# zypher-game/uzkge

Hardware: AMD Instinct MI355X
Metric: bn254_g1_msm_points_per_sec (higher is better)
Workload: dtype u256 (254-bit modular integers: 8 x u32 Montgomery limbs in HBM, 9 x 29-bit limbs in the two hot loops); 1 GPU; BN254 G1 MSM, 2^24 random points + uniform scalars per GPU, bases resident in HBM; points_per_gpu=16777216, total_points=16777216

## Files before the change

### uzkge_amd/csrc/api.cpp

```cpp
#include <algorithm>
#include <atomic>
#include <cstdarg>
#include <cstdlib>
#include <cstring>
#include <exception>
#include <new>
#include <vector>

#include "anemoi29.hpp"
#include "ctx.hpp"
#include "lane_tools.hpp"
#include "fq12_29.hpp"
#include "g16_pk_layout.hpp"
#include "g2_29.hpp"
#include "host_ec64.hpp"
#include "host_math.hpp"
#include "shufflecs_dev.hpp"
#include "matchcs_dev.hpp"

namespace uzk {

static thread_local char g_err[512] = "";

void set_error(const char* fmt, ...) {
// ... 281 lines not shown
    prover_release_all();
    vf_release_all();
    g2_release_all();
    rcs_release_all();
    g16_release_all();
    g16v_release_all();
    remark_release_all();
    std::lock_guard<std::mutex> lk(s.mu);
    if (!s.bound) return UZK_OK;
    ctx_release(default_ctx());
    for (auto& kv : s.contexts) { ctx_release(*kv.second); delete kv.second; }
    s.contexts.clear();
    s.epoch.fetch_add(1, std::memory_order_acq_rel);
    t_handle = 0;
    t_cached = nullptr;
    for (auto& kv : s.srs) {
        (void)hipSetDevice(kv.second.device);
        if (kv.second.owned && kv.second.d_points) (void)hipFree(kv.second.d_points);
        if (kv.second.d_table) (void)hipFree(kv.second.d_table);
    }
    s.srs.clear();
    s.num_cus.clear();
    s.bound = false;
    s.device = -1;
    return UZK_OK;
} catch (...) { return uzk::on_exception("uzk_shutdown"); }

namespace uzk {
static void copy_tuning(const Ctx& from, Ctx& to) {
    to.msm_window_bits = from.msm_window_bits;
    to.tune_no_precompute = from.tune_no_precompute; to.tune_ntt_tile = from.tune_ntt_tile; to.tune_ntt_two_pass = from.tune_ntt_two_pass; to.tune_small = from.tune_small;
    to.tune_chunk_log = from.tune_chunk_log; to.tune_verify_transcript = from.tune_verify_transcript; to.tune_stream_log = from.tune_stream_log; to.tune_stream_min_log = from.tune_stream_min_log;
    to.tune_seg_sort = from.tune_seg_sort; to.tune_arith29 = from.tune_arith29;
    to.tune_msm_taper = from.tune_msm_taper;
}
}
int uzk_ctx_create(uint64_t* ctx_out) try {
    if (!ctx_out) { set_error("uzk_ctx_create: null pointer"); return UZK_ERR_PARAMETER; }
    Ctx* c = new Ctx();
    {
        API_LOCK;
        int rc = require_ready();
        if (rc != UZK_OK) { delete c; return rc; }
        copy_tuning(ctx(), *c);
    }
    Shared& s = shared();
    std::lock_guard<std::mutex> lk(s.mu);
    const uint64_t h = s.next_ctx++;
    s.contexts[h] = c;
    *ctx_out = h;
    return UZK_OK;
} catch (...) { return uzk::on_exception("uzk_ctx_create"); }
int uzk_ctx_create_on(int device, uint64_t* ctx_out) try {
    if (!ctx_out) { set_error("uzk_ctx_create_on: null pointer"); return UZK_ERR_PARAMETER; }
    int n = 0;
    if (hipGetDeviceCount(&n) != hipSuccess || n <= 0) { set_error("no HIP device visible: the MI355X backend has no CPU fallback"); return UZK_ERR_DEVICE; }
    if (device < 0 || device >= n) { set_error("uzk_ctx_create_on(%d): %d device(s) visible", device, n); return UZK_ERR_PARAMETER; }
    Ctx* c = new Ctx();
    {
        API_LOCK;
        copy_tuning(ctx(), *c);
    }
    c->want_device = device;
    Shared& s = shared();
    std::lock_guard<std::mutex> lk(s.mu);
    const uint64_t h = s.next_ctx++;
    s.contexts[h] = c;
// ... 1874 lines not shown
    UZK_HIP(hipStreamSynchronize(ctx().stream));
    return UZK_OK;
} catch (...) { return uzk::on_exception("uzk_sync"); }
void* uzk_stream(void) {
    API_LOCK;
    if (require_ready() != UZK_OK) return nullptr;
    return ctx().stream;
}
int uzk_msm_set_window_bits(int c) try {
    API_LOCK;
    if (c != 0 && (c < 4 || c > 22)) { set_error("window bits must be 0 (auto) or 4..22"); return UZK_ERR_PARAMETER; }
    ctx().msm_window_bits = c;
    return UZK_OK;
} catch (...) { return uzk::on_exception("uzk_msm_set_window_bits"); }

int uzk_msm_plan_info(size_t n, int* window_bits, int* windows) try {
    API_LOCK;
    if (!window_bits || !windows || n == 0) { set_error("uzk_msm_plan_info: bad arguments"); return UZK_ERR_PARAMETER; }
    msm_plan_info(ctx(), n, window_bits, windows);
    return UZK_OK;
} catch (...) { return uzk::on_exception("uzk_msm_plan_info"); }

int uzk_tune(const char* key, int value) try {
    API_LOCK;
    if (!key) { set_error("uzk_tune: null key"); return UZK_ERR_PARAMETER; }
    Ctx& c = ctx();
    if (!std::strcmp(key, "msm_no_precompute")) c.tune_no_precompute = value;
    else if (!std::strcmp(key, "msm_stream_log")) c.tune_stream_log = (value >= -1 && value <= 26) ? value : 0;
    else if (!std::strcmp(key, "msm_stream_min_log")) c.tune_stream_min_log = (value >= 4 && value <= 26) ? value : 22;
    else if (!std::strcmp(key, "msm_chunk_log")) c.tune_chunk_log = (value >= 8 && value <= 26) ? value : 26;
    else if (!std::strcmp(key, "msm_small")) c.tune_small = value ? 1 : 0;
    else if (!std::strcmp(key, "msm_seg_sort")) c.tune_seg_sort = value;
    else if (!std::strcmp(key, "msm_taper")) c.tune_msm_taper = (value >= 0 && value <= 2) ? value : 1;
    else if (!std::strcmp(key, "ntt_tile")) c.tune_ntt_tile = (value == 1024 || value == 2048) ? value : 0;
    else if (!std::strcmp(key, "ntt_two_pass")) c.tune_ntt_two_pass = value ? 1 : 0;
    else if (!std::strcmp(key, "arith29")) c.tune_arith29 = value & 7;
    else if (!std::strcmp(key, "verify_transcript")) c.tune_verify_transcript = (value == 1 || value == 2) ? value : 0;
    else { set_error("uzk_tune: unknown key %s", key); return UZK_ERR_PARAMETER; }
    return UZK_OK;
} catch (...) { return uzk::on_exception("uzk_tune"); }

}
```

### uzkge_amd/csrc/ctx.hpp

```cpp
#pragma once
#include <hip/hip_runtime.h>

#include <cstdint>
#include <cstdlib>
#include <cstdio>
#include <chrono>
#include <map>
#include <mutex>
#include <string>
#include <vector>

#include "../../include/uzkge_gpu.h"
#include "../../include/uzkge_gpu_test.h"
#include "ec.hpp"

namespace uzk {

void set_error(const char* fmt, ...);
int on_exception(const char* fn) noexcept;

#define UZK_HIP(expr)                                                                      \
    do {                                                                                   \
        hipError_t _e = (expr);                                                            \
        if (_e != hipSuccess) {                                                            \
// ... 47 lines not shown
    bool ready = false;
    int want_device = -1;
    int device = -1;
    hipStream_t stream = nullptr;
    hipStream_t stream2 = nullptr;
    hipStream_t cur_stream = nullptr;
    int num_cus = 256;
    bool prof_on = false;
    std::vector<ProfEntry> prof_pending;
    std::vector<hipEvent_t> event_pool;
    std::map<std::string, std::pair<double, uint64_t>> prof_totals;
    std::map<uint64_t, NttPlan*> ntt_plans;
    DevBuf ntt_scratch[2];
    DevBuf ntt_io;
    MsmWork* msm = nullptr;
    DevBuf msm_scalars;
    Fp* msm_tail_host = nullptr;
    size_t msm_tail_cap = 0;
    int msm_window_bits = 0;
    int tune_no_precompute = 0;
    int tune_ntt_two_pass = 1;
    int tune_ntt_tile = 0;
    int tune_small = 1;
    int tune_chunk_log = 26;
    int tune_stream_log = 0;
    int tune_stream_min_log = 22;
    int tune_arith29 = default_arith29();
    static int default_arith29() {
        static const int v = [] { const char* e = std::getenv("UZK_ARITH29"); return e ? std::atoi(e) : 7; }();
        return v;
    }
    int tune_seg_sort = 1;
    int tune_msm_taper = 1;
    DevBuf poly_tmp, poly_tmp2, poly_io, zpoly_tmp, open_tmp, poly_args;
    DevBuf poly_cnt;
    uint32_t trim_flip = 0;
    void* poly_host = nullptr;
    size_t poly_host_cap = 0;
    DevBuf ntt_sub;
    struct PowCache { Fp key; bool valid = false; uint64_t stamp = 0; DevBuf buf; };
    PowCache pow_cache[8];
    uint64_t pow_stamp = 0;
    std::vector<void*> ntt_fused;
    std::map<uint64_t, void*> g1ntt_plans;
    DevBuf g1ntt_work, g1ntt_prefix, g1ntt_io;
    DevBuf verify_ws;
    DevBuf srs_records, srs_weights, srs_points;
    void* g2 = nullptr;
    void* g16 = nullptr;
    DevBuf g16v_ws;
    DevBuf pairing_ws;
    std::vector<uint8_t> pairing_status;
    DevBuf ed_ws;
    DevBuf ed_gen;
    bool ed_gen_ready = false;
    DevBuf shuffle_ws;
    DevBuf match_ws;
    DevBuf reveal_ws;
    DevBuf reveal_z;
    DevBuf codec_ws;
    int tune_verify_transcript = 0;
    struct Srs {
        Affine* d_points = nullptr;
        size_t n = 0;
        bool owned = false;
        int device = 0;
// ... 268 lines not shown
```

### uzkge_amd/csrc/msm.hip

```cpp
#include <algorithm>
#include <cmath>
#include <mutex>
#include <functional>
#include <memory>
#include <condition_variable>
#include <atomic>
#include <cstring>
#include <thread>
#include <vector>

#include "ctx.hpp"
#include "ec29.hpp"
#include "ecquad.hpp"
#include "ecquad29.hpp"
#include "ec29l.hpp"
#include "host_ec64.hpp"
#include "host_math.hpp"
#include "lane_tools.hpp"
#include "msm_cut.hpp"

namespace uzk {

constexpr uint32_t kSeg = 16;
constexpr uint32_t kSignBit = 0x80000000u;
constexpr uint32_t kCombineFan = 32;
constexpr int kMaxPasses = 3;

struct MsmWork {
    DevBuf digits, bucket_count, bucket_start, sorted, buckets, partials, win_sums, class_sums, big;
    DevBuf ent[2];
    DevBuf counts[kMaxPasses], segs_start[kMaxPasses], segs_len[kMaxPasses], items[kMaxPasses];
    DevBuf lvl_cnt[2], lvl_off[2], lvl_part[2], small, task_desc, exc;
    XYZZ* h_sums = nullptr;
    size_t h_sums_cap = 0;
    uint32_t* h_max = nullptr;
};

__host__ __device__ inline int msm_num_windows(int c) {
    int W = (254 + c - 1) / c;
    if (254 - (W - 1) * c == c) ++W;
    return W;
}

__device__ __forceinline__ uint32_t msm_fold_scalar_sign(Fp& k) {
    bool gt = false, decided = false;
#pragma unroll
    for (int j = 7; j >= 0; --j) {
        const uint32_t two_k = (k.v[j] << 1) | (j ? (k.v[j - 1] >> 31) : 0u);
        if (!decided && two_k != FrCfg::M[j]) { gt = two_k > FrCfg::M[j]; decided = true; }
    }
    if (!gt) return 0u;
    k = Fr::neg(k);
    return kSignBit;
}


__global__ __launch_bounds__(256) void msm_digits_kernel(ScalarView scalars, uint32_t* __restrict__ digits,
                                                         uint32_t n, uint32_t batch, int c, int W, int w0, int wcnt,
                                                         uint32_t* __restrict__ zero8 = nullptr) {
    const uint64_t t = (uint64_t)blockIdx.x * blockDim.x + threadIdx.x;
    if (zero8 != nullptr && t < 8) zero8[t] = 0;
    if (t >= (uint64_t)n * batch) return;
    const uint32_t b = (uint32_t)(t / n), i = (uint32_t)(t % n);
    Fp k = Fr::from_mont(scalars.at(b, i));
    const uint32_t flip = msm_fold_scalar_sign(k);
    const uint32_t mask = (1u << c) - 1, half = 1u << (c - 1);
    uint32_t carry = 0;
    uint32_t* dst = digits + (size_t)b * wcnt * n + i;
// ... 139 lines not shown
            if constexpr (FROM_DIGITS) {
                const uint32_t mag = a.digits[(size_t)seg * a.n + k] & ~kSignBit;
                if (mag) atomicAdd(&cnt[((mag - 1) >> a.shift) & a.mask], 1u);
            } else if constexpr (PK_IN) {
                const uint32_t e = reinterpret_cast<const uint32_t*>(a.in_entries)[(size_t)base + k];
                atomicAdd(&cnt[(pk_key(e, a.pk_in_bits) >> a.shift) & a.mask], 1u);
            } else {
                atomicAdd(&cnt[(a.in_entries[(size_t)base + k].x >> a.shift) & a.mask], 1u);
            }
        }
        __syncthreads();
        uint32_t* dst = a.counts + cidx;
        for (uint32_t b = threadIdx.x; b < a.bins; b += blockDim.x) dst[b] = cnt[b];
        if constexpr (FROM_DIGITS) return;
        __syncthreads();
    }
}

__global__ __launch_bounds__(512) void msm_radix_scan_kernel(RadixArgs a, uint32_t nch, const uint32_t* __restrict__ out_start_of,
                                                             uint32_t out_stride) {
    __shared__ uint32_t wsum[8];
    const uint32_t seg = blockIdx.x, b = threadIdx.x, G = gridDim.y, g = blockIdx.y;
    if (a.seg_min_len && a.seg_len[seg] <= a.seg_min_len) return;
    uint32_t run = 0;
    if (b < a.bins) {
        size_t first = (size_t)seg * nch;
        uint32_t cnt = nch;
        if (a.item_off) { first = a.item_off[seg]; cnt = a.item_off[seg + 1] - a.item_off[seg]; }
        const uint32_t per = (cnt + G - 1) / G;
        const uint32_t c0 = min(cnt, g * per), c1 = min(cnt, c0 + per);
        const uint32_t* p0 = a.counts + first * a.bins + b;
        uint32_t r0 = 0, r1 = 0, r2 = 0, r3 = 0;
        uint32_t ch = 0;
        for (; ch + 4 <= c0; ch += 4) {
            r0 += p0[(size_t)ch * a.bins];
            r1 += p0[(size_t)(ch + 1) * a.bins];
            r2 += p0[(size_t)(ch + 2) * a.bins];
            r3 += p0[(size_t)(ch + 3) * a.bins];
        }
        for (; ch < c0; ++ch) r0 += p0[(size_t)ch * a.bins];
        run = r0 + r1 + r2 + r3;
        for (ch = c0; ch < c1; ++ch) {
            const size_t at = (first + ch) * a.bins + b;
            const uint32_t v = a.counts[at];
            a.prefix[at] = run;
            run += v;
        }
    }
    if (g + 1 != G) return;
    uint32_t incl = run;
    for (int o = 1; o < 64; o <<= 1) {
        const uint32_t t = __shfl_up((int)incl, o);
        if ((int)(b & 63) >= o) incl += t;
    }
    if ((b & 63) == 63) wsum[b >> 6] = incl;
    __syncthreads();
    uint32_t pre = 0;
    for (uint32_t w = 0; w < (b >> 6); ++w) pre += wsum[w];
    const uint32_t excl = pre + incl - run;
    if (b < a.bins) {
        const uint32_t start = out_start_of ? out_start_of[seg] : seg * out_stride;
        a.bin_base[(size_t)seg * a.bins + b] = start + excl;
        a.bin_count[(size_t)seg * a.bins + b] = run;
    }
}

// ... 302 lines not shown
        __syncthreads();
    }
    uint32_t run = part[tid] - s;
    for (uint32_t b = lo; b < hi; ++b) {
        const uint32_t v = stage[pad(b)];
        stage[pad(b)] = run;
        run += v;
    }
    __syncthreads();
    uint32_t* off_o = off_out + (size_t)w * NB;
    uint32_t* v_o = v_out ? v_out + (size_t)w * NB : nullptr;
    for (uint32_t i = tid; i < NB; i += 1024) {
        off_o[i] = stage[pad(i)];
        if (v_o) v_o[i] = tasks(i, cnt[i]);
    }
    if (tid == 1023) win_total[w] = part[1023];
    if (max_out) {
        for (int o = 32; o > 0; o >>= 1) {
            mx = max(mx, (uint32_t)__shfl_down((int)mx, o));
            mt = max(mt, (uint32_t)__shfl_down((int)mt, o));
        }
        if ((tid & 63) == 0 && mx) { atomicMax(max_out, mx); atomicMax(max_out + 1, mt); }
    }
}
static size_t scan_win_lds(uint32_t NB) {
    static const bool raised = [] {
        return hipFuncSetAttribute(reinterpret_cast<const void*>(msm_scan_win_kernel), hipFuncAttributeMaxDynamicSharedMemorySize,
                                   ((1 << 15) + (1 << 10) + 1) * 4) == hipSuccess;
    }();
    (void)raised;
    return ((size_t)NB + NB / 32 + 1) * 4;
}
__global__ __launch_bounds__(1024) void msm_win_base_kernel(const uint32_t* __restrict__ win_total,
                                                            uint32_t* __restrict__ win_base, uint32_t W) {
    __shared__ uint32_t part[1024];
    const uint32_t tid = threadIdx.x;
    const uint32_t v = tid < W ? win_total[tid] : 0;
    part[tid] = v;
    __syncthreads();
    for (uint32_t off = 1; off < 1024; off <<= 1) {
        uint32_t t = (tid >= off) ? part[tid - off] : 0;
        __syncthreads();
        part[tid] += t;
        __syncthreads();
    }
    if (tid < W) win_base[tid] = part[tid] - v;
    if (tid == 1023) win_base[W] = part[1023];
}

__device__ __forceinline__ Affine load_point(const Affine* __restrict__ pts, uint32_t idx) {
    return pts[idx];
}

__device__ __forceinline__ void find_task(uint32_t tid, const uint32_t* __restrict__ win_base, uint32_t W,
                                          const uint32_t* __restrict__ task_off, uint32_t NB, uint32_t& w,
                                          uint32_t& b, uint32_t& j) {
    uint32_t lo = 0, hi = W;
    while (hi - lo > 1) {
        const uint32_t mid = (lo + hi) >> 1;
        if (win_base[mid] <= tid) lo = mid; else hi = mid;
    }
    w = lo;
    const uint32_t lt = tid - win_base[w];
    const uint32_t* off = task_off + (size_t)w * NB;
    lo = 0; hi = NB;
    while (hi - lo > 1) {
        const uint32_t mid = (lo + hi) >> 1;
        if (off[mid] <= lt) lo = mid; else hi = mid;
    }
    b = lo;
    j = lt - off[lo];
}

struct TaskDesc { uint32_t start, cnt, task; uint32_t pad; };
constexpr uint32_t kLenBins = 256;

__global__ __launch_bounds__(256) void msm_task_scan_kernel(const uint32_t* __restrict__ hist, uint32_t* __restrict__ cursor) {
    __shared__ uint32_t h[kLenBins];
    h[threadIdx.x] = hist[threadIdx.x];
    __syncthreads();
// ... 906 lines not shown
}

static int choose_window_bits(size_t n, int forced) {
    if (forced >= 4 && forced <= 22) return forced;
    int lg = 0;
    while ((1ull << (lg + 1)) <= n) ++lg;
    if (lg <= 16) return 8;
    if (lg <= 18) return 15;
    if (lg <= 20) return 16;
    return 17;
}
int msm_precompute_window_bits(size_t n, int forced) {
    if (forced >= 4 && forced <= 24) return forced;
    if (n <= (1u << 15)) return n <= 256 ? 5 : n <= 2048 ? 7 : 8;
    int lg = 0;
    while ((1ull << (lg + 1)) <= n) ++lg;
    return std::max(8, std::min(22, lg - 2));
}

void msm_free(Ctx& c) {
    if (!c.msm) return;
    for (int q = 0; q < 2; ++q) {
        MsmWork* m = &c.msm[q];
        m->digits.release(); m->bucket_count.release(); m->bucket_start.release(); m->sorted.release();
        m->buckets.release(); m->partials.release(); m->win_sums.release(); m->class_sums.release(); m->big.release(); m->small.release(); m->task_desc.release(); m->exc.release();
        for (int k = 0; k < 2; ++k) {
            m->ent[k].release(); m->lvl_cnt[k].release(); m->lvl_off[k].release(); m->lvl_part[k].release();
        }
        for (int k = 0; k < kMaxPasses; ++k) {
            m->counts[k].release(); m->segs_start[k].release(); m->segs_len[k].release(); m->items[k].release();
        }
        if (m->h_sums) (void)hipHostFree(m->h_sums);
        if (m->h_max) (void)hipHostFree(m->h_max);
    }
    delete[] c.msm;
    c.msm = nullptr;
    if (c.stream2) { (void)hipStreamDestroy(c.stream2); c.stream2 = nullptr; }
}

int msm_build_table(Ctx& c, const Affine* d_points, size_t n, int cb, Affine** table_out, uint32_t* W_out) {
    const uint32_t W = (uint32_t)msm_num_windows(cb);
    if ((uint64_t)W * n >= (1ull << 31)) {
        set_error("precompute: W*n = %llu exceeds 2^31 - 1", (unsigned long long)W * n);
        return UZK_ERR_PARAMETER;
    }
    Affine* table = nullptr;
    UZK_HIP(hipMalloc(reinterpret_cast<void**>(&table), (size_t)W * n * sizeof(Affine)));
    Fp *tz = nullptr, *tp = nullptr;
    hipError_t e = hipMalloc(reinterpret_cast<void**>(&tz), n * sizeof(Fp));
    if (e == hipSuccess) e = hipMalloc(reinterpret_cast<void**>(&tp), n * sizeof(Fp));
    if (e == hipSuccess) e = hipMemcpyAsync(table, d_points, n * sizeof(Affine), hipMemcpyDeviceToDevice, c.stream);
    if (e == hipSuccess && n <= (1u << 16) && W > 1) {
        (void)hipFree(tz); (void)hipFree(tp); tz = tp = nullptr;
        e = hipMalloc(reinterpret_cast<void**>(&tz), (size_t)W * n * sizeof(Fp));
        if (e == hipSuccess) e = hipMalloc(reinterpret_cast<void**>(&tp), (size_t)W * n * sizeof(Fp));
        if (e == hipSuccess) {
            KernelScope ks(c, "msm_precompute");
            hipLaunchKernelGGL(msm_precompute_column_kernel, dim3((unsigned)((n + 63) / 64)), dim3(64), 0, c.stream, table, tz, tp,
                               (uint32_t)n, cb, W);
        }
        if (e == hipSuccess) e = hipGetLastError();
        if (e == hipSuccess) e = hipStreamSynchronize(c.stream);
    } else if (e == hipSuccess) {
        const uint32_t threads = (uint32_t)((n + kPreRun - 1) / kPreRun);
        for (uint32_t j = 1; j < W; ++j) {
            KernelScope ks(c, "msm_precompute");
            hipLaunchKernelGGL(msm_precompute_kernel, dim3((threads + 63) / 64), dim3(64), 0, c.stream,
                               table + (size_t)(j - 1) * n, table + (size_t)j * n, tz, tp, (uint32_t)n, cb);
        }
        e = hipGetLastError();
        if (e == hipSuccess) e = hipStreamSynchronize(c.stream);
    }
    if (tz) (void)hipFree(tz);
    if (tp) (void)hipFree(tp);
    if (e != hipSuccess) {
        (void)hipFree(table);
        set_error("precompute failed: %s", hipGetErrorString(e));
        return UZK_ERR_DEVICE;
    }
    *table_out = table;
    *W_out = W;
    return UZK_OK;
}

struct SortPass { uint32_t shift, bins, nseg, nch, chunk, items_bound; };
constexpr int kSegCfgs = 6;
constexpr uint32_t kSegCap[kSegCfgs] = {128 * 12, 256 * 12, 256 * 24, 256 * 40, 512 * 40, 512 * 72};

struct MsmGroup {
    MsmWork* m = nullptr;
    hipStream_t st = nullptr;
    bool pre = false;
    int cb = 0;
    uint32_t W_total = 0, w0 = 0, W = 0, n32 = 0, batch = 0;
    uint64_t per_poly = 0, entries = 0, TBK = 0, bound0 = 0, part_cap = 0;
    uint32_t kb = 0, NBL = 0, S0 = 0, seg_n = 0, NB = 0, Wd = 0, RW = 0, seg = 0, groups = 0, L = 0;
    int P = 0;
    bool scan_reduce = false, quad_reduce = false;
    bool direct = false;
    uint32_t class_s = 0, nb2 = 0;
    uint32_t rl = 256;
    uint32_t pk_bits = 0;
    MsmCut cut;
    SortPass sp[kMaxPasses];
    uint32_t *cnt_cur = nullptr, *off_cur = nullptr, *base_cur = nullptr;
    XYZZ* part_cur = nullptr;
};

static int msm_group_admit(size_t n, uint32_t batch, int cb, bool pre, uint32_t W, uint32_t* NB_out, uint32_t* Wd_out) {
    const uint64_t per_poly = n < (1ull << 31) ? (uint64_t)W * n : 1ull << 31;
    if (per_poly >= (1ull << 31) || per_poly * batch >= (1ull << 31)) { set_error("msm: batch*W*n overflows the 31-bit index space"); return UZK_ERR_PARAMETER; }
    const uint32_t NBL = 1u << (cb - 1), S0 = pre ? batch : batch * W;
    uint32_t NB = std::min<uint32_t>(NBL, 1u << 15);
    while (((uint64_t)S0 * NBL) / NB > 1024 && NB < (1u << 15)) NB <<= 1;
    const uint64_t Wd = ((uint64_t)S0 * NBL) / NB;
    if (Wd > 1024) { set_error("msm: too many bucket windows (%llu): lower the batch", (unsigned long long)Wd); return UZK_ERR_PARAMETER; }
    if (NB_out) *NB_out = NB;
    if (Wd_out) *Wd_out = (uint32_t)Wd;
    return UZK_OK;
}

static int msm_group_plan(Ctx& c, MsmGroup& g, size_t n, uint32_t batch, int cb, bool pre, uint32_t W_total, uint32_t w0,
                          uint32_t W, uint64_t idx_span = 0) {
    g.pre = pre; g.cb = cb; g.W_total = W_total; g.w0 = w0; g.W = W; g.n32 = (uint32_t)n; g.batch = batch;
    UZK_TRY(msm_group_admit(n, batch, cb, pre, W, &g.NB, &g.Wd));
    g.per_poly = (uint64_t)W * n;
    g.entries = g.per_poly * batch;
    g.kb = (uint32_t)cb - 1;
    g.NBL = 1u << g.kb;
    g.S0 = pre ? batch : batch * W;
    g.seg_n = pre ? (uint32_t)g.per_poly : g.n32;
    g.TBK = (uint64_t)g.Wd * g.NB;
// ... 53 lines not shown
    }
    MsmWork& m = *g.m;
    UZK_TRY(m.digits.reserve((size_t)g.entries * 4));
    UZK_TRY(m.sorted.reserve((size_t)g.entries * 4));
    UZK_TRY(m.bucket_count.reserve((size_t)g.TBK * 4));
    UZK_TRY(m.bucket_start.reserve((size_t)g.TBK * 4));
    UZK_TRY(m.buckets.reserve((size_t)g.TBK * sizeof(XYZZ)));
    UZK_TRY(m.partials.reserve((size_t)2 * g.RW * std::max<uint32_t>(g.groups, g.class_s ? 2 * (g.nb2 / 256 + 1) : 0) * sizeof(XYZZ)));
    UZK_TRY(m.win_sums.reserve((size_t)g.RW * 2 * sizeof(XYZZ)));
    if (g.class_s) UZK_TRY(m.class_sums.reserve((size_t)g.RW * 2 * g.nb2 * sizeof(XYZZ)));
    for (int p = 0; p < g.P; ++p) {
        UZK_TRY(m.counts[p].reserve((size_t)(p == 0 ? 2 * g.sp[p].nseg * g.sp[p].nch : g.sp[p].items_bound) * g.sp[p].bins * 4));
        if (p > 0) UZK_TRY(m.items[p].reserve(((size_t)g.sp[p].nseg + 1) * 4));
        if (p + 1 < g.P) {
            UZK_TRY(m.segs_start[p].reserve((size_t)g.sp[p].nseg * g.sp[p].bins * 4));
            UZK_TRY(m.segs_len[p].reserve((size_t)g.sp[p].nseg * g.sp[p].bins * 4));
            UZK_TRY(m.ent[p & 1].reserve((size_t)g.entries * sizeof(uint2)));
        }
    }
    for (int k = 0; k < 2; ++k) {
        UZK_TRY(m.lvl_cnt[k].reserve((size_t)g.TBK * 4));
        UZK_TRY(m.lvl_off[k].reserve((size_t)g.TBK * 4));
    }
    UZK_TRY(m.lvl_part[0].reserve((size_t)g.part_cap * sizeof(XYZZ)));
    UZK_TRY(m.small.reserve(16384));
    UZK_TRY(m.task_desc.reserve((size_t)g.bound0 * sizeof(TaskDesc)));
    UZK_TRY(m.exc.reserve((size_t)g.bound0 * 4));
    if (m.h_sums_cap < (size_t)g.RW * 2) {
        if (m.h_sums) (void)hipHostFree(m.h_sums);
        UZK_HIP(hipHostMalloc(reinterpret_cast<void**>(&m.h_sums), (size_t)g.RW * 2 * sizeof(XYZZ), hipHostMallocDefault));
        m.h_sums_cap = (size_t)g.RW * 2;
    }
    if (!m.h_max) UZK_HIP(hipHostMalloc(reinterpret_cast<void**>(&m.h_max), 64, hipHostMallocDefault));
    return UZK_OK;
}

static int msm_group_phase1(Ctx& c, MsmGroup& g, const Affine* points, const ScalarView& d_scalars, uint32_t pre_stride,
                            uint32_t pre_off, bool direct_ok = true) {
    MsmWork& m = *g.m;
    hipStream_t st = g.st;
    c.cur_stream = st;
    uint32_t* digits = m.digits.as<uint32_t>();
    uint32_t* sorted = m.sorted.as<uint32_t>();
    uint32_t* bcount = m.bucket_count.as<uint32_t>();
    uint32_t* bstart = m.bucket_start.as<uint32_t>();
    uint32_t* sm = m.small.as<uint32_t>();
    uint32_t* win_tot = sm;
    uint32_t* d_max = sm + 3200;
    UZK_HIP(hipMemsetAsync(d_max, 0, (3912 - 3200) * 4, st));
    const bool fused_hist = !g.pre && g.w0 == 0 && g.W == g.W_total && g.sp[0].nch >= 256 &&
                            (size_t)g.W * g.sp[0].bins * 4 <= 64 * 1024;
    if (fused_hist) {
        KernelScope ks(c, "msm_digits");
        hipLaunchKernelGGL(msm_digits_hist_kernel, dim3(g.sp[0].nch, g.batch), dim3(1024), (size_t)g.W * g.sp[0].bins * 4, st,
                           d_scalars, digits, g.n32, g.cb, (int)g.W, g.sp[0].shift, g.sp[0].bins, m.counts[0].as<uint32_t>());
    } else {
        KernelScope ks(c, "msm_digits");
        const uint64_t tot = (uint64_t)g.n32 * g.batch;
        hipLaunchKernelGGL(msm_digits_kernel, dim3((unsigned)((tot + 255) / 256)), dim3(256), 0, st, d_scalars, digits, g.n32,
                           g.batch, g.cb, (int)g.W_total, (int)g.w0, (int)g.W, (uint32_t*)nullptr);
    }
    for (int p = 0; p < g.P; ++p) {
        const bool first = (p == 0), last = (p == g.P - 1);
        const SortPass& sp = g.sp[p];
        RadixArgs a{};
        a.shift = sp.shift; a.bins = sp.bins; a.mask = sp.bins - 1;
// ... 63 lines not shown
        }
        {
            KernelScope ks(c, "msm_sort_scan");
            const uint32_t scan_g = first ? std::max<uint32_t>(1, std::min<uint32_t>(sp.nch / 16, 1024 / std::max<uint32_t>(1, sp.nseg))) : 1u;
            hipLaunchKernelGGL(msm_radix_scan_kernel, dim3(sp.nseg, scan_g), dim3(512), 0, st, a, sp.nch,
                               first ? (const uint32_t*)nullptr : a.seg_start, first ? g.seg_n : 0u);
        }
        {
            KernelScope ks(c, "msm_sort_scatter");
            const uint32_t cs0 = first ? (g.seg_n + sp.nch - 1) / sp.nch : 0u;
            if (first && !last && a.pk_out_bits && sp.bins <= 512 && cs0 <= 32768 && !g.pre)
                hipLaunchKernelGGL((msm_radix_chunk_kernel<512, 64, 18176>), grid, dim3(512), 0, st, a);
            else if (first && last) hipLaunchKernelGGL((msm_radix_scatter_kernel<1024, 8, true, true, false>), grid, dim3(1024), 0, st, a);
            else if (first && g.entries >= (1ull << 26))
                hipLaunchKernelGGL((msm_radix_scatter_kernel<512, 8, true, false, false>), grid, dim3(512), 0, st, a);
            else if (first) hipLaunchKernelGGL((msm_radix_scatter_kernel<1024, 8, true, false, false>), grid, dim3(1024), 0, st, a);
            else if (last && a.pk_in_bits) hipLaunchKernelGGL((msm_radix_scatter_kernel<512, 8, false, true, true>), grid, dim3(512), 0, st, a);
            else if (last) hipLaunchKernelGGL((msm_radix_scatter_kernel<256, 16, false, true, false>), grid, dim3(256), 0, st, a);
            else hipLaunchKernelGGL((msm_radix_scatter_kernel<1024, 8, false, false, false>), grid, dim3(1024), 0, st, a);
        }
    }
    g.cnt_cur = m.lvl_cnt[0].as<uint32_t>();
    g.off_cur = m.lvl_off[0].as<uint32_t>();
    g.base_cur = sm + 1024;
    g.part_cur = m.lvl_part[0].as<XYZZ>();
    uint32_t* len_hist = sm + 3328;
    uint32_t* len_cur = sm + 3328 + kLenBins;
    g.direct = direct_ok;
    XYZZ* direct_buckets = g.direct ? m.buckets.as<XYZZ>() : nullptr;
    {
        KernelScope ks(c, "msm_scan_win");
        hipLaunchKernelGGL(msm_scan_win_kernel, dim3(g.Wd), dim3(1024), scan_win_lds(g.NB), st, bcount, g.L, g.cnt_cur, g.off_cur, win_tot,
                           d_max, g.NB, len_hist, g.cut);
        hipLaunchKernelGGL(msm_win_base_kernel, dim3(1), dim3(1024), 0, st, win_tot, g.base_cur, g.Wd);
    }
    TaskDesc* desc = m.task_desc.as<TaskDesc>();
    {
        KernelScope ks(c, "msm_task_order");
        uint32_t* big_count = sm + 3908;
        UZK_TRY(m.big.reserve((size_t)(g.TBK + 1) * sizeof(BigBucket)));
        hipLaunchKernelGGL(msm_task_scan_kernel, dim3(1), dim3(256), 0, st, len_hist, len_cur);
        hipLaunchKernelGGL(msm_bucket_fill_kernel, dim3((unsigned)((g.TBK + 255) / 256)), dim3(256), 0, st, g.base_cur, g.cnt_cur, g.off_cur,
                           bstart, bcount, g.NB, g.TBK, len_cur, desc, big_count, m.big.as<BigBucket>(), g.direct ? 1u : 0u, g.cut);
        hipLaunchKernelGGL(msm_task_fill_big_kernel, dim3(1024), dim3(64), 0, st, big_count, m.big.as<BigBucket>(), len_cur, desc);
    }
    {
        KernelScope ks(c, "msm_accumulate");
        const dim3 grid((unsigned)((g.bound0 + 255) / 256));
        uint32_t* exc_count = sm + 3900;
        uint32_t* exc_list = m.exc.as<uint32_t>();
        hipLaunchKernelGGL(msm_accumulate29_kernel, grid, dim3(256), 0, st, points, sorted, desc, g.base_cur, g.part_cur,
                           g.Wd, exc_count, exc_list, direct_buckets);
        hipLaunchKernelGGL(msm_accumulate_exc_kernel, dim3(std::min<unsigned>(grid.x, 128u)), dim3(256), 0, st, points, sorted, desc, g.part_cur,
                           exc_count, exc_list, direct_buckets);
    }
    UZK_HIP(hipGetLastError());
    UZK_HIP(hipMemcpyAsync(m.h_max, d_max, 8, hipMemcpyDeviceToHost, st));
    return UZK_OK;
}

static int msm_group_phase2(Ctx& c, MsmGroup& g, bool accumulate = false, bool reduce = true) {
    const int a29 = (c.tune_arith29 >> 2) & 1;
    MsmWork& m = *g.m;
    hipStream_t st = g.st;
    c.cur_stream = st;
    UZK_HIP(hipStreamSynchronize(st));
    uint32_t* sm = m.small.as<uint32_t>();
    uint32_t* win_tot = sm;
    uint32_t* win_base[2] = {sm + 1024, sm + 2080};
    XYZZ* buckets = m.buckets.as<XYZZ>();
    XYZZ* partials = m.partials.as<XYZZ>();
    XYZZ* win_sums = m.win_sums.as<XYZZ>();
    const uint32_t G = kCombineFan;
    static_assert(kCutMaxTasks <= kCombineFan, "a short-cut bucket must never need a fold level of its own");
    uint64_t tmax = m.h_max[1];
    const uint32_t gs = g.TBK >= (1u << 18) ? 1u : (tmax > 2 ? 4u : 1u);
    constexpr uint32_t kBigThresh = 4;
    static_assert(sizeof(BigFold) == sizeof(BigBucket), "the two lists share one buffer");
    const bool big_mode = gs == 1 && tmax > kBigThresh;
    uint32_t* big_count = sm + 3904;
    BigFold* big_list = nullptr;
    if (big_mode) {
        UZK_TRY(m.big.reserve((size_t)(g.bound0 / G + g.TBK + 1) * sizeof(BigFold)));
        big_list = m.big.as<BigFold>();
    }
    if (g.direct && tmax > G) {
        KernelScope ks(c, "msm_combine");
        hipLaunchKernelGGL(msm_undirect_kernel, dim3((unsigned)((g.TBK + 255) / 256)), dim3(256), 0, st, buckets, g.cnt_cur, g.off_cur,
                           g.base_cur, g.part_cur, g.NB, g.TBK);
        g.direct = false;
    }
    if (accumulate && g.direct) { set_error("msm: direct bucket writes in an accumulating chunk (internal error)"); return UZK_ERR_DEVICE; }
    const int skip_single = g.direct ? 1 : 0;
    int lvl = 0;
    uint64_t bound_prev = g.bound0;
    const MsmCut fin_cut = tmax > G ? MsmCut() : g.cut;
    while (tmax > G) {
        const int nx = (lvl + 1) & 1;
        UZK_TRY(m.lvl_part[nx].reserve((size_t)g.part_cap * sizeof(XYZZ)));
        uint32_t* cnt_nx = m.lvl_cnt[nx].as<uint32_t>();
        uint32_t* off_nx = m.lvl_off[nx].as<uint32_t>();
        uint32_t* base_nx = win_base[nx];
        const uint64_t bound_nx = bound_prev / G + g.TBK;
        XYZZ* part_nx = m.lvl_part[nx].as<XYZZ>();
        {
            KernelScope ks(c, "msm_scan_win");
            hipLaunchKernelGGL(msm_scan_win_kernel, dim3(g.Wd), dim3(1024), scan_win_lds(g.NB), st, g.cnt_cur, G, cnt_nx, off_nx, win_tot,
                               (uint32_t*)nullptr, g.NB);
            hipLaunchKernelGGL(msm_win_base_kernel, dim3(1), dim3(1024), 0, st, win_tot, base_nx, g.Wd);
        }
        {
            KernelScope ks(c, "msm_combine");
            const dim3 grid((unsigned)((bound_nx * gs + 255) / 256));
            if (gs == 16)
                hipLaunchKernelGGL(msm_combine_kernel<16>, grid, dim3(256), 0, st, g.part_cur, g.cnt_cur, g.off_cur, g.base_cur,
                                   off_nx, base_nx, part_nx, g.NB, g.Wd, G, (uint32_t*)nullptr, (BigFold*)nullptr, 0u, a29);
            else if (gs == 4)
                hipLaunchKernelGGL(msm_combine_kernel<4>, grid, dim3(256), 0, st, g.part_cur, g.cnt_cur, g.off_cur, g.base_cur,
                                   off_nx, base_nx, part_nx, g.NB, g.Wd, G, (uint32_t*)nullptr, (BigFold*)nullptr, 0u, a29);
            else {
                if (big_mode) UZK_HIP(hipMemsetAsync(big_count, 0, 4, st));
                hipLaunchKernelGGL(msm_combine_kernel<1>, grid, dim3(256), 0, st, g.part_cur, g.cnt_cur, g.off_cur, g.base_cur,
                                   off_nx, base_nx, part_nx, g.NB, g.Wd, G, big_count, big_list, kBigThresh, a29);
                if (big_mode)
                    hipLaunchKernelGGL(msm_fold_big_kernel, dim3(2048), dim3(64), 0, st, g.part_cur, big_count, big_list, part_nx, 0);
            }
        }
        g.cnt_cur = cnt_nx; g.off_cur = off_nx; g.base_cur = base_nx; g.part_cur = part_nx;
        bound_prev = bound_nx;
        tmax = (tmax + G - 1) / G;
        lvl = nx;
    }
// ... 260 lines not shown
            const uint64_t lanes = cap[k] * (uint64_t)gs * (quad ? 4 : 1);
            const dim3 grid((unsigned)((lanes + 255) / 256));
            const SmallChunk* cd = cdesc + lv.dbase[k];
#define UZK_FOLD(QD, G) hipLaunchKernelGGL((msm_small_fold_kernel<QD, G>), grid, dim3(256), 0, st, P, cd, counters + k, lv.pbase[k], (c.tune_arith29 >> 2) & 1)
            if (quad) { if (gs >= 8) UZK_FOLD(true, 8); else if (gs >= 4) UZK_FOLD(true, 4); else UZK_FOLD(true, 2); }
            else { if (gs >= 8) UZK_FOLD(false, 8); else if (gs >= 4) UZK_FOLD(false, 4); else if (gs >= 2) UZK_FOLD(false, 2); else UZK_FOLD(false, 1); }
#undef UZK_FOLD
        }
        {
            KernelScope ks(c, "msm_small_reduce");
            const uint32_t Q = std::min<uint32_t>(NBL, 64);
            if ((c.tune_arith29 >> 2) & 1) hipLaunchKernelGGL((msm_small_reduce_kernel<3, 256>), dim3(S), dim3(4 * Q), (size_t)Q * 144, st, P, bucket_ref, cdesc,
                               slot_chunks, lv, win_sums, NBL);
            else hipLaunchKernelGGL((msm_small_reduce_kernel<2, 256>), dim3(S), dim3(4 * Q), (size_t)Q * 144, st, P, bucket_ref, cdesc,
                               slot_chunks, lv, win_sums, NBL);
        }
        UZK_HIP(hipGetLastError());
    }
    {
        HostScope hs(c, "host_msm_wait2");
        UZK_HIP(hipStreamSynchronize(st));
    }
    auto window_sum = [&](uint32_t b, uint32_t w) -> const XYZZ& { return m.h_sums[(size_t)b * W + w]; };
    msm_horner_host(c, batch, W, pre_c > 0 ? 0 : cb, window_sum, out_host);
    return UZK_OK;
}

int msm_run_streamed(Ctx& c, const Affine* points, const Fp* scalars_host, size_t n, Jac* out_host) {
    if (!c.msm) c.msm = new MsmWork[2];
    const int cb = choose_window_bits(n, c.msm_window_bits);
    const uint32_t W = (uint32_t)msm_num_windows(cb);
    std::vector<size_t> bounds{0};
    {
        const size_t cap = (size_t)1 << (c.tune_stream_log > 0 ? std::max(16, std::min(26, c.tune_stream_log)) : 22);
        size_t sz = c.tune_stream_log > 0 ? cap : std::min<size_t>(cap, (size_t)1 << 20);
        int at_this_size = 0;
        while (bounds.back() < n) {
            bounds.push_back(std::min(n, bounds.back() + sz));
            if (++at_this_size >= (sz == ((size_t)1 << 20) ? 2 : 1) && sz < cap) { sz <<= 1; at_this_size = 0; }
        }
    }
    const size_t nchunks = bounds.size() - 1;
    size_t chunk = 0;
    for (size_t k = 0; k < nchunks; ++k) chunk = std::max(chunk, bounds[k + 1] - bounds[k]);
    if (!c.stream2) UZK_HIP(hipStreamCreateWithFlags(&c.stream2, hipStreamNonBlocking));
    hipStream_t copy_st = c.stream2;
    UZK_TRY(c.msm_scalars.reserve(2 * chunk * sizeof(Fp)));
    Fp* stage[2] = {c.msm_scalars.as<Fp>(), c.msm_scalars.as<Fp>() + chunk};
    hipEvent_t up_done[2] = {c.get_event(), c.get_event()}, consumed[2] = {c.get_event(), c.get_event()};
    auto give_back = [&] { for (int i = 0; i < 2; ++i) { c.event_pool.push_back(up_done[i]); c.event_pool.push_back(consumed[i]); } };
    MsmGroup g;
    g.m = &c.msm[0];
    g.st = c.stream;
    int rc = UZK_OK;
    auto upload = [&](size_t k) -> int {
        const size_t lo = bounds[k], len = bounds[k + 1] - lo;
        const int s = (int)(k & 1);
        if (k >= 2) UZK_HIP(hipStreamWaitEvent(copy_st, consumed[s], 0));
        HostScope hs(c, "host_msm_upload");
        UZK_HIP(hipMemcpyAsync(stage[s], scalars_host + lo, len * sizeof(Fp), hipMemcpyHostToDevice, copy_st));
        UZK_HIP(hipEventRecord(up_done[s], copy_st));
        return UZK_OK;
    };
    rc = msm_group_plan(c, g, chunk, 1, cb, false, W, 0, W);
    if (rc == UZK_OK) rc = upload(0);
    for (size_t k = 0; k < nchunks && rc == UZK_OK; ++k) {
        const size_t lo = bounds[k], len = bounds[k + 1] - lo;
// ... 99 lines not shown
```

Measured before the change: 886.8 million points/s.

## Signal bucket max to host early via mapped write and event instead of stream sync

The win-base kernel now copies the device max counts straight into pinned host memory. An event is recorded after that kernel, so the host waits only on the event rather than synchronizing the whole stream after the task-order and accumulate kernels. This lets host planning for the reduction overlap with the remaining bucket accumulation, and buffer growth falls back to a full stream sync to avoid reallocating memory that kernels may still be using. It also adds a 16-way unrolled accumulator to a count-summing loop and lowers the minimum stream chunk log from 16 to 13.

```diff
diff --git a/uzkge_amd/csrc/api.cpp b/uzkge_amd/csrc/api.cpp
--- a/uzkge_amd/csrc/api.cpp
+++ b/uzkge_amd/csrc/api.cpp
@@ -337,7 +337,7 @@
     to.tune_no_precompute = from.tune_no_precompute; to.tune_ntt_tile = from.tune_ntt_tile; to.tune_ntt_two_pass = from.tune_ntt_two_pass; to.tune_small = from.tune_small;
     to.tune_chunk_log = from.tune_chunk_log; to.tune_verify_transcript = from.tune_verify_transcript; to.tune_stream_log = from.tune_stream_log; to.tune_stream_min_log = from.tune_stream_min_log;
     to.tune_seg_sort = from.tune_seg_sort; to.tune_arith29 = from.tune_arith29;
-    to.tune_msm_taper = from.tune_msm_taper;
+    to.tune_msm_taper = from.tune_msm_taper; to.tune_msm_early = from.tune_msm_early;
 }
 }
 int uzk_ctx_create(uint64_t* ctx_out) try {
@@ -2278,6 +2278,7 @@
     else if (!std::strcmp(key, "msm_small")) c.tune_small = value ? 1 : 0;
     else if (!std::strcmp(key, "msm_seg_sort")) c.tune_seg_sort = value;
     else if (!std::strcmp(key, "msm_taper")) c.tune_msm_taper = (value >= 0 && value <= 2) ? value : 1;
+    else if (!std::strcmp(key, "msm_early")) c.tune_msm_early = (value >= 0 && value <= 2) ? value : 1;
     else if (!std::strcmp(key, "ntt_tile")) c.tune_ntt_tile = (value == 1024 || value == 2048) ? value : 0;
     else if (!std::strcmp(key, "ntt_two_pass")) c.tune_ntt_two_pass = value ? 1 : 0;
     else if (!std::strcmp(key, "arith29")) c.tune_arith29 = value & 7;
diff --git a/uzkge_amd/csrc/ctx.hpp b/uzkge_amd/csrc/ctx.hpp
--- a/uzkge_amd/csrc/ctx.hpp
+++ b/uzkge_amd/csrc/ctx.hpp
@@ -103,6 +103,7 @@
     }
     int tune_seg_sort = 1;
     int tune_msm_taper = 1;
+    int tune_msm_early = 1;
     DevBuf poly_tmp, poly_tmp2, poly_io, zpoly_tmp, open_tmp, poly_args;
     DevBuf poly_cnt;
     uint32_t trim_flip = 0;
diff --git a/uzkge_amd/csrc/msm.hip b/uzkge_amd/csrc/msm.hip
--- a/uzkge_amd/csrc/msm.hip
+++ b/uzkge_amd/csrc/msm.hip
@@ -34,6 +34,7 @@
     XYZZ* h_sums = nullptr;
     size_t h_sums_cap = 0;
     uint32_t* h_max = nullptr;
+    hipEvent_t ev_max = nullptr;
 };
 
 __host__ __device__ inline int msm_num_windows(int c) {
@@ -239,6 +240,13 @@
         const uint32_t* p0 = a.counts + first * a.bins + b;
         uint32_t r0 = 0, r1 = 0, r2 = 0, r3 = 0;
         uint32_t ch = 0;
+        uint32_t r[16] = {};
+        for (; ch + 16 <= c0; ch += 16) {
+#pragma unroll
+            for (uint32_t j = 0; j < 16; ++j) r[j] += p0[(size_t)(ch + j) * a.bins];
+        }
+#pragma unroll
+        for (uint32_t j = 0; j < 16; ++j) r0 += r[j];
         for (; ch + 4 <= c0; ch += 4) {
             r0 += p0[(size_t)ch * a.bins];
             r1 += p0[(size_t)(ch + 1) * a.bins];
@@ -607,7 +615,9 @@
     return ((size_t)NB + NB / 32 + 1) * 4;
 }
 __global__ __launch_bounds__(1024) void msm_win_base_kernel(const uint32_t* __restrict__ win_total,
-                                                            uint32_t* __restrict__ win_base, uint32_t W) {
+                                                            uint32_t* __restrict__ win_base, uint32_t W,
+                                                            const uint32_t* __restrict__ max_in = nullptr,
+                                                            uint32_t* __restrict__ max_host = nullptr) {
     __shared__ uint32_t part[1024];
     const uint32_t tid = threadIdx.x;
     const uint32_t v = tid < W ? win_total[tid] : 0;
@@ -621,6 +631,7 @@
     }
     if (tid < W) win_base[tid] = part[tid] - v;
     if (tid == 1023) win_base[W] = part[1023];
+    if (max_host && tid < 2) { max_host[tid] = max_in[tid]; __threadfence_system(); }
 }
 
 __device__ __forceinline__ Affine load_point(const Affine* __restrict__ pts, uint32_t idx) {
@@ -1593,6 +1604,7 @@
         }
         if (m->h_sums) (void)hipHostFree(m->h_sums);
         if (m->h_max) (void)hipHostFree(m->h_max);
+        if (m->ev_max) c.event_pool.push_back(m->ev_max);
     }
     delete[] c.msm;
     c.msm = nullptr;
@@ -1659,6 +1671,7 @@
     int P = 0;
     bool scan_reduce = false, quad_reduce = false;
     bool direct = false;
+    bool early_max = false;
     uint32_t class_s = 0, nb2 = 0;
     uint32_t rl = 256;
     uint32_t pk_bits = 0;
@@ -1778,6 +1791,7 @@
         m.h_sums_cap = (size_t)g.RW * 2;
     }
     if (!m.h_max) UZK_HIP(hipHostMalloc(reinterpret_cast<void**>(&m.h_max), 64, hipHostMallocDefault));
+    if (!m.ev_max) m.ev_max = c.get_event();
     return UZK_OK;
 }
 
@@ -1907,8 +1921,11 @@
         KernelScope ks(c, "msm_scan_win");
         hipLaunchKernelGGL(msm_scan_win_kernel, dim3(g.Wd), dim3(1024), scan_win_lds(g.NB), st, bcount, g.L, g.cnt_cur, g.off_cur, win_tot,
                            d_max, g.NB, len_hist, g.cut);
-        hipLaunchKernelGGL(msm_win_base_kernel, dim3(1), dim3(1024), 0, st, win_tot, g.base_cur, g.Wd);
-    }
+        g.early_max = c.tune_msm_early != 0;
+        hipLaunchKernelGGL(msm_win_base_kernel, dim3(1), dim3(1024), 0, st, win_tot, g.base_cur, g.Wd,
+                           g.early_max ? (const uint32_t*)d_max : (const uint32_t*)nullptr, g.early_max ? m.h_max : (uint32_t*)nullptr);
+    }
+    if (g.early_max) UZK_HIP(hipEventRecord(m.ev_max, st));
     TaskDesc* desc = m.task_desc.as<TaskDesc>();
     {
         KernelScope ks(c, "msm_task_order");
@@ -1930,7 +1947,7 @@
                            exc_count, exc_list, direct_buckets);
     }
     UZK_HIP(hipGetLastError());
-    UZK_HIP(hipMemcpyAsync(m.h_max, d_max, 8, hipMemcpyDeviceToHost, st));
+    if (!g.early_max) UZK_HIP(hipMemcpyAsync(m.h_max, d_max, 8, hipMemcpyDeviceToHost, st));
     return UZK_OK;
 }
 
@@ -1939,7 +1956,12 @@
     MsmWork& m = *g.m;
     hipStream_t st = g.st;
     c.cur_stream = st;
-    UZK_HIP(hipStreamSynchronize(st));
+    if (g.early_max) UZK_HIP(hipEventSynchronize(m.ev_max));
+    else UZK_HIP(hipStreamSynchronize(st));
+    auto reserve_idle = [&](DevBuf& b, size_t bytes) -> int {
+        if (bytes > b.cap && g.early_max) UZK_HIP(hipStreamSynchronize(st));
+        return b.reserve(bytes);
+    };
     uint32_t* sm = m.small.as<uint32_t>();
     uint32_t* win_tot = sm;
     uint32_t* win_base[2] = {sm + 1024, sm + 2080};
@@ -1956,7 +1978,7 @@
     uint32_t* big_count = sm + 3904;
     BigFold* big_list = nullptr;
     if (big_mode) {
-        UZK_TRY(m.big.reserve((size_t)(g.bound0 / G + g.TBK + 1) * sizeof(BigFold)));
+        UZK_TRY(reserve_idle(m.big, (size_t)(g.bound0 / G + g.TBK + 1) * sizeof(BigFold)));
         big_list = m.big.as<BigFold>();
     }
     if (g.direct && tmax > G) {
@@ -1972,7 +1994,7 @@
     const MsmCut fin_cut = tmax > G ? MsmCut() : g.cut;
     while (tmax > G) {
         const int nx = (lvl + 1) & 1;
-        UZK_TRY(m.lvl_part[nx].reserve((size_t)g.part_cap * sizeof(XYZZ)));
+        UZK_TRY(reserve_idle(m.lvl_part[nx], (size_t)g.part_cap * sizeof(XYZZ)));
         uint32_t* cnt_nx = m.lvl_cnt[nx].as<uint32_t>();
         uint32_t* off_nx = m.lvl_off[nx].as<uint32_t>();
         uint32_t* base_nx = win_base[nx];
@@ -2299,7 +2321,7 @@
     const uint32_t W = (uint32_t)msm_num_windows(cb);
     std::vector<size_t> bounds{0};
     {
-        const size_t cap = (size_t)1 << (c.tune_stream_log > 0 ? std::max(16, std::min(26, c.tune_stream_log)) : 22);
+        const size_t cap = (size_t)1 << (c.tune_stream_log > 0 ? std::max(13, std::min(26, c.tune_stream_log)) : 22);
         size_t sz = c.tune_stream_log > 0 ? cap : std::min<size_t>(cap, (size_t)1 << 20);
         int at_this_size = 0;
         while (bounds.back() < n) {
```

Result: no change. 889.8 million points/s (median of 6 runs) (+0.3%).
